# alv-around/mini-stark

Measured on AMD Instinct MI355X. Metric: stark_proofs_per_s, higher is better.
Workload: dtype u64; 1 GPU; Fibonacci AIR, Goldilocks, 2^20 trace rows, blowup 8, 20 security bits (w=3, c=6, rounds=23, ood_queries=1, fri_queries=2); a step = 8 independent proofs in flight per GPU

## Files before the change

mini-stark_amd/csrc/ctx.hpp:

```cpp
#pragma once
#include "../../include/ministark.h"

#include <cstdarg>
#include <cstdio>
#include <cstdlib>
#include <map>
#include <new>
#include <string>
#include <type_traits>
#include <vector>

#include "field.hpp"
#include "merkle.hpp"
#include "ntt.hpp"
#include "poly.hpp"

namespace msctx {

struct DevBuf {
  void* p = nullptr; size_t cap = 0;
  int ensure(size_t bytes) {
    if (bytes <= cap) return 0;
    if (p) msrt::free_dev(p);
    p = nullptr; cap = 0;
    size_t want = bytes + bytes / 8 + 256;
    if (msrt::malloc_dev(&p, want)) { p = nullptr; return 1; }
    cap = want;
    return 0;
  }
  void release() { if (p) msrt::free_dev(p); p = nullptr; cap = 0; }
// ... 112 lines not shown
  void drop_rccl();
  void unshard() { sh_on = false; sh_rank = 0; sh_world = 1; xs = xr = nullptr; xcap = 0; xfn = nullptr; xuser = nullptr; have_lde = false; nrounds_done = 0; blob_size = 0; }
  int set_shard_rccl(int rank, int world, const u8* unique_id, size_t cap) override;
  int rccl_selftest() override;
  int shard_proof_on_root(int on) override { proof_root_only = on ? 1 : 0; return MS_OK; }
  int shard_proof_is_elsewhere() const override { return (proof_root_only && sh_world > 1 && sh_rank != 0 && nrounds_done == fri_rounds && fri_rounds) ? 1 : 0; }
  int shard_round_is_distributed(int r) override { return (r >= 0 && (size_t)r < nrounds_done && rounds[r]->dist) ? 1 : 0; }
  int shard_stats(u64* out) override { if (!out) return fail(MS_ERR_ARG, "shard_stats"); memcpy(out, xstat, sizeof xstat); return MS_OK; }
  bool shardable(size_t leaf_groups) const { return sh_on && leaf_groups >= shard_min_leaves && leaf_groups >= (size_t)sh_world * (size_t)sh_world; }
  int set_shard(int rank, int world, void* d_send, void* d_recv, size_t cap, ms_exchange_fn fn, void* user) override;

  int fail_rt(int e, const char* what) { err = std::string("runtime error ") + std::to_string(e) + " in " + what + ": " + msrt::last_error_string(); return MS_ERR_HIP; }
  int fail(int code, const char* msg) { err = msg; return code; }

  enum { K_NTT_PASS, K_SCALE_POW, K_LEAF_HASH, K_INNER_HASH, K_TRANSPOSE, K_IO, K_LINCOMB, K_MIX, K_EVAL, K_EVAL_REDUCE, K_FOLD,
         K_SUFFIX_HORNER, K_DEGREE, K_FIND_FIRST, K_PATH, K_QUERY_POINTS, K_FRI_TAIL, K_COUNT };
  struct ProfRec { int kid, sub; msrt::Event* a; msrt::Event* b; double bytes; bool part; };
  int part_depth = 0;
  struct PartScope { Ctx* c; explicit PartScope(Ctx* c_) : c(c_) { c->part_depth++; } ~PartScope() { c->part_depth--; } };
  struct PartScopeIf { Ctx* c; bool on; PartScopeIf(Ctx* c_, bool on_) : c(c_), on(on_) { if (on) c->part_depth++; } ~PartScopeIf() { if (on) c->part_depth--; } };
  bool prof_on = false;
  std::vector<ProfRec> prof_recs;
  double next_bytes = 0;
  int next_sub = 0;
  std::vector<std::string> ntt_names{std::string("?")};
  void name_next(const char* fmt, ...) __attribute__((format(printf, 2, 3))) {
    if (!prof_on) return;
    char buf[200]; va_list ap; va_start(ap, fmt); vsnprintf(buf, sizeof buf, fmt, ap); va_end(ap);
    for (size_t i = 0; i < ntt_names.size(); i++) if (ntt_names[i] == buf) { next_sub = (int)i; return; }
    ntt_names.push_back(buf); next_sub = (int)ntt_names.size() - 1;
  }
// ... 23 lines not shown
    prof_recs.push_back(r);
    return e;
  }
  template <class K> int run(int kid, unsigned gx, unsigned gy, int threads, size_t lds, const typename K::Params& p) {
    launched();
    if (gx == 0 || gy == 0) return 0;
    if (!prof_on) return msrt::launch<K>(stream, gx, gy, threads, lds, p);
    ProfRec r; r.kid = kid; r.sub = next_sub; r.bytes = next_bytes; r.part = part_depth > 0; next_bytes = 0; next_sub = 0;
    if (msrt::event_create(&r.a) || msrt::event_create(&r.b)) return 1;
    msrt::event_record(r.a, stream);
    int e = msrt::launch<K>(stream, gx, gy, threads, lds, p);
    msrt::event_record(r.b, stream);
    prof_recs.push_back(r);
    return e;
  }
  int profile_begin() override { prof_on = true; return 0; }
  int profile_end(char* out, size_t cap) override;

  struct Plan {
    int log_n = 0, log_r0 = 0, log_rho = 0, npass = 0, K[4] = {0, 0, 0, 0}, lo_bits = 0;
    int LC[4] = {msntt::TILE_LOG_C, msntt::TILE_LOG_C, msntt::TILE_LOG_C, msntt::TILE_LOG_C};
    bool v2[4] = {false, false, false, false};
    bool regp[4] = {false, false, false, false};
    DevBuf tw_lo, tw_hi, w_r[4], vtw, w0;
    T n_inv = 0;
  };
  std::map<int, Plan*> plans;
  DevBuf ntt_scratch;
  int ntt_kmax = 9;
  int ntt_v2 = 1, ntt_v2_regpass = 1;
  int ntt_fast = 1;
// ... 182 lines not shown
  int sh_launch_inline(const SHJ& j, int final_mode);
  int sh_launch_table(const SHJ* d_jobs, size_t njobs, size_t maxnb, int final_mode);
  int shard_carry_table(const mspoly::CarryJob<F, E>* d_jobs, size_t njobs);
  int suffix_horner(const T* in, size_t in_limb_stride, size_t in_off, size_t in_stride, size_t m, const XE& z,
                    T* out, size_t out_limb_stride, size_t out_off, size_t out_stride, T* h0);

  int gather_poly(const T* local, size_t S, size_t count, T* dst, size_t dst_stride);
  int fold_dist(Round* pr, Round* nr, const XE& a, size_t* nq_coef_out);
  int fri_fold_commit(const u64* alpha, u8* root) override;
  size_t fri_tail_max = (size_t)1 << 15;
  int fri_overlap = 0;
  msrt::Stream* side_stream = nullptr; msrt::Event* ev_side = nullptr; bool side_pending = false;
  struct StreamScope { Ctx* c; msrt::Stream* keep; StreamScope(Ctx* c_, msrt::Stream* s) : c(c_), keep(c_->stream) { c->stream = s; } ~StreamScope() { c->stream = keep; } };
  int join_side() { if (side_pending) { side_pending = false; CK(msrt::stream_wait_event(stream, ev_side)); } return 0; }
  int fri_tail_round(Round* pr, Round* nr, const XE& a, bool* done);
  template <class DG> int fri_tail_round_t(Round* pr, Round* nr, const XE& a, bool* done);
  int fri_round_info(int r, u64* ncoef, u64* D) override;
  int fri_round_poly_read(int r, u64* out) override;
  int fri_round_codeword_read(int r, u64* out) override;

  bool blob_external = false;
  int fri_query(const u64* betas, int nq, u8* ext_out, size_t ext_cap, size_t* ext_len) override;
  struct QueryPlan {
    typedef mspoly::CarryJob<F, E> CJ; typedef mspoly::FindJob<F, E> FJ; typedef msmerkle::PathJob<F, E> PJ; typedef msmerkle::ShardPathJob<F, E> SPJ;
    size_t W = 0; int nq = 0; size_t pos = 0; u8* blob = nullptr;
    T* d_h0 = nullptr; T* d_tg = nullptr; unsigned long long* d_ix = nullptr;
    std::vector<size_t> rec_off, path_off; std::vector<u64> qlen; std::vector<T> x1h;
    std::vector<std::vector<SHJ>> tables; std::vector<int> table_mode, table_part; size_t n_agg_tables = 0;
    std::vector<CJ> carry_jobs; bool any_dist = false;
    std::vector<msmerkle::CopyJob> unp; std::vector<size_t> unp_first, unp_cnt, chunk_c0, chunk_len;
// ... 39 lines not shown
```

mini-stark_amd/csrc/fri_commit.cpp:

```cpp
#include "ctx.hpp"
#include "fri_tail.hpp"

namespace msctx {

template <class F>
int Ctx<F>::round_commit(Round* r, size_t ncoef_in, int nonzero_limbs, const Round* prev, const XE* alpha) {
  if (ctz64(r->D) > F::TWO_ADICITY) return fail(MS_ERR_SHAPE, "FRI domain larger than the field's two-adicity");
  RQ(tree_shape(r->D, 2, 2, &r->ts));
  r->m = 0;
  {
    const bool shard_next = shardable(r->D / 2);
    bool z_outside_base = false;
    for (int l = 1; l < E; l++) z_outside_base = z_outside_base || cur_z.c[l] != 0;
    if (prev && fri_pointwise && z_outside_base && prev->D == 2 * r->D && prev->ts.sharded == shard_next) {
      Plan* pl;
      RQ(get_plan(ctz64(prev->D), 0, false, &pl));
      const size_t W = (size_t)sh_world;
      const size_t m_out = shard_next ? r->D / (2 * W) : r->D;
      const size_t local = shard_next ? 2 * m_out : r->D;
      if (shard_next) r->m = m_out;
      if (r->cw.ensure(local * E * sizeof(T))) return fail(MS_ERR_NOMEM, "codeword");
      const size_t total = m_out * (shard_next ? 2 : 1);
      const XE c = e_add<F, E>(cur_B[0], e_mul<F>(cur_B[1], *alpha));
      auto fold_launch = [&](auto* kernel) {
        typedef typename std::remove_pointer<decltype(kernel)>::type FK;
        typename FK::Params fp;
        fp.src = prev->cw.template as<T>(); fp.src_limb_stride = shard_next ? 2 * prev->m : prev->D;
        fp.dst = r->cw.template as<T>(); fp.dst_limb_stride = local;
        fp.m_out = m_out; fp.log_m = (u32)ctz64(m_out); fp.groups = shard_next ? 2 : 1; fp.shard_W = shard_next ? (u32)W : 0; fp.shard_k = (u32)sh_rank;
        fp.tw_lo = pl->tw_lo.template as<T>(); fp.tw_hi = pl->tw_hi.template as<T>(); fp.lo_bits = (u32)pl->lo_bits; fp.log_D = (u32)ctz64(prev->D);
        fp.alpha = *alpha;
        fp.c2 = e_add<F, E>(c, c);
        fp.z = cur_z;
        fp.inv2 = f_inv<F>(F::from_u64(2));
        return run<FK>(K_FOLD, grid1(total, FK::THREADS * FK::ITEMS), 1, FK::THREADS, 0, fp);
      };
      next_bytes = (double)total * E * sizeof(T) * 3;
      { PartScopeIf part(this, shard_next); CK(total <= fold_small_max ? fold_launch((mspoly::FriFoldEvalKernel<F, E, 1>*)nullptr) : fold_launch((mspoly::FriFoldEvalKernel<F, E, 8>*)nullptr)); }
      if (shard_next) RQ((tree_build_sharded<E>(r->cw.template as<T>(), m_out, 1, 2 * m_out, 2, r->ts, r->nodes)));
      else RQ((tree_build<E>(r->cw.template as<T>(), 0, 1, r->D, 1, r->ts, r->nodes)));
      return 0;
    }
  }
  RQ(join_side());
  if (shardable(r->D / 2)) {
    const size_t m = r->D / (2 * (size_t)sh_world);
    r->m = m;
    if (r->cw.ensure(2 * m * E * sizeof(T))) return fail(MS_ERR_NOMEM, "codeword");
    const T* coef = r->poly.template as<T>(); size_t coef_stride = r->cap;
// ... 273 lines not shown
  u32 nl = 0; while (((size_t)1 << nl) < per) nl++;
  tp.sub.nodes = nr->nodes.template as<u32>(); tp.sub.child_off = 0; tp.sub.nchildren = M; tp.sub.ic = 2; tp.sub.nlevels = nl;
  u32 tl = 0; while (((size_t)1 << tl) < G) tl++;
  tp.top.nodes = nr->nodes.template as<u32>(); tp.top.child_off = 2 * M - 2 * G; tp.top.nchildren = G; tp.top.ic = 2; tp.top.nlevels = tl;
  tp.top.host_root = host_root(); tp.top.aux_src = dres; tp.top.aux_dst = reinterpret_cast<unsigned long long*>(pinned); tp.top.flag = arm_flag();
  tp.root_index = nr->ts.nodes - 1;
  tp.done = reinterpret_cast<u32*>(d_deg.as<u8>() + 128);
  next_bytes = (double)Dn * E * sizeof(T) * 3 + (double)M * 96;
  CK(run_coop<TK>(K_FRI_TAIL, (unsigned)(G + 1), TK::THREADS, TK::lds_bytes(), tp));
  root_on_host = true; aux_on_host = true;
  *done = true;
  return 0;
}

template <class F>
int Ctx<F>::fri_fold_commit(const u64* alpha, u8* root) {
  if (!have_deep) return fail(MS_ERR_STATE, "fri_fold_commit before fri_deep");
  XE a;
  if (!alpha || !root || !load_ext(alpha, &a)) return fail(MS_ERR_ARG, "alpha");
  Round* pr = rounds[nrounds_done - 1];
  if (pr->D < 4) return fail(MS_ERR_SHAPE, "FRI round domain too small to fold (merkle.rs:93-104 panics)");
  const size_t n = pr->ncoef, m = (n + 1) / 2;
  Round* nr = round_slot(nrounds_done);
  nr->cap = m ? m : 1;
  nr->D = pr->D / 2;
  nr->dist = false; nr->local_store = false; nr->S = 0;
  size_t nq_coef = 0;
  bool fused = false, side = false;
  RQ(fri_tail_round(pr, nr, a, &fused));
  if (fused) {
    CK(sync_results());
    nr->ncoef = (size_t)(*reinterpret_cast<unsigned long long*>(pinned));
    memcpy(root, reinterpret_cast<const u8*>(host_root()), 32);
    nrounds_done++; have_deep = false;
    return MS_OK;
  }
  if (pr->dist) RQ(fold_dist(pr, nr, a, &nq_coef));
  else {
  if (nr->poly.ensure(nr->cap * E * sizeof(T)) || d_folded.ensure((m + 1) * E * sizeof(T))) return fail(MS_ERR_NOMEM, "fold");
  if (m >= 2) {
    side = fri_overlap && !prof_on;
    if (side && !side_stream) { CK(msrt::stream_create(&side_stream)); CK(msrt::event_create(&ev_side)); }
    StreamScope on_side(this, side ? side_stream : stream);
    typename mspoly::FoldKernel<F, E>::Params fp{pr->poly.template as<T>(), pr->cap, n, d_folded.as<T>(), m, a, nullptr};
    CK(run<mspoly::FoldKernel<F, E>>(K_FOLD, grid1(m, mspoly::THREADS), 1, mspoly::THREADS, 0, fp));
    RQ(suffix_horner(d_folded.as<T>(), m, 0, 1, m, cur_z, nr->poly.template as<T>(), nr->cap, 0, 1, nullptr));
    nq_coef = m - 1;
  }
  }
  unsigned long long* dres = d_deg.as<unsigned long long>();
  if (nr->dist) {
    const size_t lc = lcount(nr, nq_coef);
    if (lc) {
      typename mspoly::DegreeKernel<F, E>::Params dp{lpoly(nr), lstride(nr), lc, dres, (size_t)sh_rank * nr->S};
      PartScope part(this);
      CK(run<mspoly::DegreeKernel<F, E>>(K_DEGREE, grid1(lc, mspoly::THREADS), 1, mspoly::THREADS, 0, dp));
    }
    shard_aux = dres;
  } else if (nq_coef) {
    StreamScope on_side(this, side ? side_stream : stream);
    typename mspoly::DegreeKernel<F, E>::Params dp{nr->poly.template as<T>(), nr->cap, nq_coef, dres, 0};
    CK(run<mspoly::DegreeKernel<F, E>>(K_DEGREE, grid1(nq_coef, mspoly::THREADS), 1, mspoly::THREADS, 0, dp));
  }
  if (side) { CK(msrt::event_record(ev_side, side_stream)); side_pending = true; }
  pending_aux = dres; aux_on_host = false;
  { auto clear = scope_exit([this] { pending_aux = nullptr; shard_aux = nullptr; });
    auto join = scope_exit([this] { if (side_pending) { side_pending = false; seq_armed = 0; msrt::stream_wait_event(stream, ev_side); } });
    RQ(round_commit(nr, nq_coef, E, pr, &a)); }
  if (!aux_on_host) { seq_armed = 0; CK(msrt::d2h(pinned, dres, 8, stream)); CK(msrt::memset_dev(dres, 0, 8, stream)); }
  if (!root_on_host) { seq_armed = 0; CK(msrt::d2h(reinterpret_cast<u8*>(pinned) + 64, nr->nodes.template as<u8>() + (nr->ts.local_nodes - 1) * 32, 32, stream)); }
  CK(sync_results());
  nr->ncoef = (size_t)(*reinterpret_cast<unsigned long long*>(pinned));
  memcpy(root, root_on_host ? reinterpret_cast<const u8*>(host_root()) : reinterpret_cast<const u8*>(pinned) + 64, 32);
  nrounds_done++; have_deep = false;
  return MS_OK;
}

template <class F>
int Ctx<F>::fri_round_info(int r, u64* ncoef, u64* D) {
  if (r < 0 || (size_t)r >= nrounds_done) return fail(MS_ERR_ARG, "round index");
  if (ncoef) *ncoef = rounds[r]->ncoef;
// ... 17 lines not shown

#define MS_INSTANTIATE(FF) \
  template int Ctx<FF>::round_commit(Ctx<FF>::Round* r, size_t ncoef_in, int nonzero_limbs, const Ctx<FF>::Round* prev, const Ctx<FF>::XE* alpha); \
  template int Ctx<FF>::degree_launch(const Ctx<FF>::T* poly, size_t limb_stride, size_t n, unsigned long long** dres_out); \
  template int Ctx<FF>::read_degree_and_root(const Ctx<FF>::T* poly, size_t limb_stride, size_t n, Ctx<FF>::Round* r, size_t* ncoef, u8* root); \
  template int Ctx<FF>::fri_begin(size_t blowup_, size_t nrounds, u8* root0); \
  template int Ctx<FF>::fri_deep(const u64* z, u64* B); \
  template Ctx<FF>::SHPlan Ctx<FF>::sh_plan(const Ctx<FF>::T* in, size_t in_limb_stride, size_t in_off, size_t in_stride, size_t m, const Ctx<FF>::XE& z, void* out, bool out_u64, size_t out_limb_stride, size_t out_off, size_t out_stride, Ctx<FF>::T* h0, Ctx<FF>::T* scratch, const Ctx<FF>::T* ext_carry, Ctx<FF>::T* top_agg, bool out_h0); \
  template int Ctx<FF>::sh_launch_inline(const Ctx<FF>::SHJ& j, int final_mode); \
  template int Ctx<FF>::sh_launch_table(const Ctx<FF>::SHJ* d_jobs, size_t njobs, size_t maxnb, int final_mode); \
  template int Ctx<FF>::shard_carry_table(const mspoly::CarryJob<FF, Ctx<FF>::E>* d_jobs, size_t njobs); \
  template int Ctx<FF>::suffix_horner(const Ctx<FF>::T* in, size_t in_limb_stride, size_t in_off, size_t in_stride, size_t m, const Ctx<FF>::XE& z, Ctx<FF>::T* out, size_t out_limb_stride, size_t out_off, size_t out_stride, Ctx<FF>::T* h0); \
  template int Ctx<FF>::gather_poly(const Ctx<FF>::T* local, size_t S, size_t count, Ctx<FF>::T* dst, size_t dst_stride); \
  template int Ctx<FF>::fold_dist(Ctx<FF>::Round* pr, Ctx<FF>::Round* nr, const Ctx<FF>::XE& a, size_t* nq_coef_out); \
  template int Ctx<FF>::fri_tail_round(Ctx<FF>::Round* pr, Ctx<FF>::Round* nr, const Ctx<FF>::XE& a, bool* done); \
  template int Ctx<FF>::fri_fold_commit(const u64* alpha, u8* root); \
  template int Ctx<FF>::fri_round_info(int r, u64* ncoef, u64* D); \
  template int Ctx<FF>::fri_round_poly_read(int r, u64* out); \
  template int Ctx<FF>::fri_round_codeword_read(int r, u64* out);
MS_INSTANTIATE(GL)
MS_INSTANTIATE(BB)
#undef MS_INSTANTIATE

}
```

mini-stark_amd/csrc/merkle_tree.cpp:

```cpp
#include "ctx.hpp"
#include "blake2s.hpp"

namespace msctx {

template <class F>
int Ctx<F>::tree_shape(size_t leaf_num, size_t lpn, size_t ic, TreeShape* ts) {
  if (lpn == 0 || ic < 2 || !is_pow2(ic)) return fail(MS_ERR_SHAPE, "merkle: bad leafs_per_node / inner_children");
  const size_t node_num = leaf_num / lpn;
  long lg = log_two_k(node_num, ic);
  if (lg < 0) return fail(MS_ERR_SHAPE, lg == -1 ? "number if not a power of 2" : "number if not a power of base");
  if (leaf_num % lpn != 0) return fail(MS_ERR_SHAPE, "merkle: leaf_num % leafs_per_node != 0");
  if (lg >= 64 || node_num == 0) return fail(MS_ERR_SHAPE, "Tree is not full!");
  ts->leaf_num = leaf_num; ts->lpn = lpn; ts->ic = ic; ts->levels = (size_t)lg + 1;
  size_t total = 0, m = node_num;
  for (;;) { total += m; if (m == 1) break; m /= ic; }
  ts->nodes = total; ts->local_nodes = total; ts->Mloc = 0; ts->sharded = false;
  return 0;
}

template <class F> template <int EL>
int Ctx<F>::leaf_hash(const T* base, size_t col_stride, size_t row_stride, size_t limb_stride, u32 width, size_t lpn, size_t ngroups, u32* out,
              size_t g_first, u32 run_len, u32 run_stride, const msmerkle::LinColSpec* lin, size_t out_g0) {
  if (ngroups >> 32) return fail(MS_ERR_SHAPE, "more than 2^32 leaf groups");
  if (digest == MS_DIGEST_BLAKE2S256) {
// ... 66 lines not shown
  auto to_rec = [&](msmerkle::InnerHashKernel::Params& ip) {
    ip.host_root = reinterpret_cast<u32*>(rec_out);
    if (shard_aux) { ip.aux_src = shard_aux; ip.aux_dst = reinterpret_cast<unsigned long long*>(rec_out + 32); }
    rec_done = true;
  };
  const bool b2 = digest == MS_DIGEST_BLAKE2S256;
  while (nchildren > 1) {
    msmerkle::InnerHashKernel::Params ip;
    ip.nodes = nodes; ip.child_off = child_off; ip.nchildren = nchildren; ip.ic = (u32)ic; ip.host_root = nullptr; ip.aux_src = nullptr; ip.aux_dst = nullptr; ip.flag = msrt::HostFlag{nullptr, 0};
    const size_t nparents = nchildren / ic;
    if (ic == 2 && nparents <= subtree_parents && (nchildren & (nchildren - 1)) == 0) {
      typedef msmerkle::InnerSubtreeKernel SK;
      u32 nl = 0; for (size_t m = nchildren; m > 1 && nl < (u32)SK::MAX_LEVELS; m >>= 1) nl++;
      const size_t left = nchildren >> nl;
      if (final_levels && left == 1) {
        RQ(join_side());
        ip.host_root = host_root(); root_on_host = true;
        if (pending_aux) { ip.aux_src = pending_aux; ip.aux_dst = reinterpret_cast<unsigned long long*>(pinned); pending_aux = nullptr; aux_on_host = true; }
        ip.flag = arm_flag();
      } else if (rec_out && left == 1) to_rec(ip);
      ip.nlevels = nl;
      next_bytes = (double)nchildren * 32 * 2;
      if (b2) CK(run_coop<msmerkle::B2InnerSubtreeKernel>(K_INNER_HASH, (unsigned)left, SK::THREADS, SK::lds_bytes(), ip));
      else CK(run_coop<SK>(K_INNER_HASH, (unsigned)left, SK::THREADS, SK::lds_bytes(), ip));
      for (u32 l = 0; l < nl; l++) { child_off += nchildren; nchildren >>= 1; }
      continue;
    }
    if (final_levels && (nparents == 1 || nparents <= (size_t)tree_top_parents)) {
      RQ(join_side());
      ip.host_root = host_root(); root_on_host = true;
      if (pending_aux) { ip.aux_src = pending_aux; ip.aux_dst = reinterpret_cast<unsigned long long*>(pinned); pending_aux = nullptr; aux_on_host = true; }
      ip.flag = arm_flag();
    } else if (rec_out && (nparents == 1 || nparents <= (size_t)tree_top_parents)) to_rec(ip);
    if (nparents <= (size_t)tree_top_parents) {
      u32 nl = 0; for (size_t m = nchildren; m > 1; m /= ic) nl++;
      ip.nlevels = nl;
      next_bytes = (double)nchildren * 32 * 2;
      RQ(inner_launch(1, ip));
      break;
    }
    ip.nlevels = 1;
    next_bytes = (double)nparents * (ic * 32 + 32);
    RQ(inner_launch((unsigned)((nparents + msmerkle::THREADS - 1) / msmerkle::THREADS), ip));
    child_off += nchildren; nchildren = nparents;
  }
  if (rec_out && !rec_done) {
    CK(msrt::d2d(rec_out, reinterpret_cast<u8*>(nodes) + (child_off + nchildren - 1) * 32, 32, stream));
    if (shard_aux) CK(msrt::d2d(rec_out + 32, shard_aux, 8, stream)); else CK(msrt::memset_dev(rec_out + 32, 0, 8, stream));
  }
  return 0;
}

template <class F> template <int EL>
int Ctx<F>::tree_build_sharded(const T* base, size_t col_stride, size_t row_stride, size_t limb_stride, u32 width, TreeShape& ts, DevBuf& nodes, const msmerkle::LinColSpec* lin) {
  const size_t W = (size_t)sh_world, M = ts.leaf_num / ts.lpn, Mloc = M / W, per = Mloc / W;
  if (ts.ic != 2 || per == 0) return fail(MS_ERR_STATE, "sharded tree needs a binary tree with at least world^2 leaf groups");
  if (Mloc * 32 > xcap) return fail(MS_ERR_NOMEM, "exchange buffers too small for the sharded commitment (need 32 * leaf groups / world bytes)");
  const size_t sub_nodes = 2 * Mloc - 1, top_nodes = 2 * W - 1;
// ... 110 lines not shown
```

mini-stark_amd/csrc/rt.hpp:

```cpp
#pragma once
#include <cstddef>
#include <cstdint>
#include <cstring>

#if defined(MS_HOST_ONLY)
#define MS_HD inline
#define MS_DEV inline
#define MS_RESTRICT
MS_HD uint64_t ms_mulhi64(uint64_t a, uint64_t b) { return (uint64_t)(((unsigned __int128)a * b) >> 64); }

#elif defined(MS_EMU)
#include <cstdlib>
#include <vector>
#define MS_HD inline
#define MS_DEV inline
#define MS_RESTRICT
namespace msrt {
struct Stream { int dummy; };
inline int malloc_dev(void** p, size_t n) { *p = std::malloc(n ? n : 1); return *p ? 0 : 1; }
inline int free_dev(void* p) { std::free(p); return 0; }
inline int malloc_host(void** p, size_t n) { *p = std::malloc(n ? n : 1); return *p ? 0 : 1; }
inline int malloc_host_coherent(void** p, size_t n) { return malloc_host(p, n); }
inline int free_host(void* p) { std::free(p); return 0; }
inline int h2d(void* d, const void* h, size_t n, Stream*) { std::memcpy(d, h, n); return 0; }
// ... 163 lines not shown
  return r;
}
template <class K> struct CoopArgs { const typename K::Params* p; int bx, by, nbx, threads; unsigned char* lds; };
template <class K> inline void coop_entry(void* a, int tid) { auto* c = (CoopArgs<K>*)a; K::run(*c->p, c->bx, c->by, c->nbx, tid, c->lds); }
template <class K>
inline int launch_coop(Stream*, unsigned gx, unsigned gy, int threads, size_t lds_bytes, const typename K::Params& p) {
  static thread_local FiberBlock fb;
  std::vector<unsigned char> lds(lds_bytes + 16);
  for (unsigned by = 0; by < gy; by++)
    for (unsigned bx = 0; bx < gx; bx++) {
      CoopArgs<K> a{&p, (int)bx, (int)by, (int)gx, threads, lds.data()};
      fb.run_block(threads, &coop_entry<K>, &a);
    }
  return 0;
}
MS_DEV void atomic_min_u64(unsigned long long* a, unsigned long long v) { if (v < *a) *a = v; }
MS_DEV void atomic_max_u64(unsigned long long* a, unsigned long long v) { if (v > *a) *a = v; }
MS_DEV unsigned atomic_add_u32(unsigned* a, unsigned v) { unsigned o = *a; *a = o + v; return o; }
MS_DEV unsigned wave_alloc_slot(unsigned* counter, bool want) { if (!want) return 0; unsigned o = *counter; *counter = o + 1; return o; }
MS_DEV bool wave_any(bool pred) { return pred; }
inline unsigned pair_swap(unsigned v) { return (unsigned)wave_shfl_xor(v, 7); }
inline unsigned pair_exchange_add(bool a_lane, unsigned v, unsigned t, unsigned s) {
  const unsigned long long r = wave_shfl_xor((unsigned long long)v | ((unsigned long long)t << 32), 7);
  return a_lane ? (unsigned)(r >> 32) + s : (unsigned)r + t;
}
inline unsigned rotr_var(unsigned x, unsigned r) { return (x >> r) | (x << ((32 - r) & 31)); }
struct HostFlag { unsigned long long* dst; unsigned long long val; };
MS_DEV void raise_host_flag(const HostFlag& f) { if (f.dst) *f.dst = f.val; }
inline void raise_host_flag_wg(const HostFlag& f, int tid) { if (f.dst && tid == 0) *f.dst = f.val; }
}
// ... 275 lines not shown
template <class K>
__global__ void __launch_bounds__(K::THREADS, MinWaves<K>::v) ms_kmain_coop(const typename K::Params p) {
  extern __shared__ __align__(16) unsigned char ms_lds[];
  K::run(p, (int)blockIdx.x, (int)blockIdx.y, (int)gridDim.x, (int)threadIdx.x, ms_lds);
}
template <class K>
inline int launch_coop(Stream* s, unsigned gx, unsigned gy, int threads, size_t lds_bytes, const typename K::Params& p) {
  if (threads != K::THREADS) return (int)hipErrorInvalidValue;
  if (lds_bytes > 65536) {
    hipError_t e = hipFuncSetAttribute(reinterpret_cast<const void*>(&ms_kmain_coop<K>), hipFuncAttributeMaxDynamicSharedMemorySize, (int)lds_bytes);
    if (e != hipSuccess) return (int)e;
  }
  hipLaunchKernelGGL(HIP_KERNEL_NAME(ms_kmain_coop<K>), dim3(gx, gy, 1), dim3(threads, 1, 1), lds_bytes, s, p);
  return (int)hipGetLastError();
}

MS_DEV void wg_barrier() { asm volatile("s_waitcnt lgkmcnt(0)\n\ts_barrier" ::: "memory"); }
MS_DEV void wg_barrier_global() { __syncthreads(); }
MS_DEV void fence_device() { __threadfence(); }
MS_DEV unsigned long long wave_shfl_xor(unsigned long long v, int mask) { return __shfl_xor(v, mask, 64); }
MS_DEV int wave_uniform(int v) { return __builtin_amdgcn_readfirstlane(v); }
MS_DEV void atomic_min_u64(unsigned long long* a, unsigned long long v) { atomicMin(a, v); }
MS_DEV void atomic_max_u64(unsigned long long* a, unsigned long long v) { atomicMax(a, v); }
MS_DEV unsigned atomic_add_u32(unsigned* a, unsigned v) { return atomicAdd(a, v); }
MS_DEV bool wave_any(bool pred) { return __any(pred) != 0; }
MS_DEV unsigned wave_alloc_slot(unsigned* counter, bool want) {
  const unsigned long long mask = __ballot(want);
  if (!want) return 0;
  const unsigned lane = __lane_id();
  const int leader = __ffsll((long long)mask) - 1;
// ... 51 lines not shown
```

mini-stark_amd/csrc/session.cpp:

```cpp
#include "ctx.hpp"

namespace msctx {

template <class F>
int Ctx<F>::profile_end(char* out, size_t cap) {
  static const char* names[K_COUNT] = {"ntt_pass", "scale_pow", "leaf_hash", "inner_hash", "transpose_in", "io_copy", "lincomb", "mix", "eval", "eval_reduce",
                                       "fold", "suffix_horner", "degree", "find_first", "merkle_path", "query_points", "fri_tail"};
  msrt::sync(stream);
  double ms[K_COUNT] = {0}, by[K_COUNT] = {0}, ms_part = 0, ms_repl = 0, repl_by[K_COUNT] = {0}; unsigned long long cnt[K_COUNT] = {0};
  std::map<int, double> sub_ms, sub_by; std::map<int, unsigned long long> sub_cnt;
  for (auto& r : prof_recs) {
    float t = 0.f; msrt::event_elapsed_ms(&t, r.a, r.b);
    ms[r.kid] += t; by[r.kid] += r.bytes; cnt[r.kid]++;
    if (r.part) ms_part += t; else { ms_repl += t; repl_by[r.kid] += t; }
    if (r.kid == K_NTT_PASS) { sub_ms[r.sub] += t; sub_by[r.sub] += r.bytes; sub_cnt[r.sub]++; }
    msrt::event_destroy(r.a); msrt::event_destroy(r.b);
  }
  prof_recs.clear(); prof_on = false;
  std::string j = "{";
  for (int k = 0; k < K_COUNT; k++) {
    char buf[256];
    snprintf(buf, sizeof buf, "%s\"%s\": {\"launches\": %llu, \"ms\": %.6f, \"alg_bytes\": %.0f}", k ? ", " : "", names[k], cnt[k], ms[k], by[k]);
    j += buf;
  }
  j += ", \"ntt_pass_variants\": {";
  bool first = true;
  for (auto& kv : sub_ms) {
    const int sub = kv.first; char buf[420];
    const char* name = ntt_names[(size_t)sub < ntt_names.size() ? sub : 0].c_str();
    snprintf(buf, sizeof buf, "%s\"%s\": {\"launches\": %llu, \"ms\": %.6f, \"alg_bytes\": %.0f}", first ? "" : ", ", name, sub_cnt[sub], kv.second, sub_by[sub]);
    j += buf; first = false;
  }
  j += "}";
// ... 58 lines not shown
  digest = (flags & MS_FLAG_DIGEST_BLAKE2S) ? MS_DIGEST_BLAKE2S256 : MS_DIGEST_SHA256;
  if (const char* e = getenv("MS_NTT_KMAX")) { int v = atoi(e); if (v >= 5 && v <= msntt::MAX_LOG_R) ntt_kmax = v; }
  if (const char* e = getenv("MS_NTT_FAST")) ntt_fast = atoi(e);
  if (const char* e = getenv("MS_NTT_V2")) ntt_v2 = atoi(e);
  if (const char* e = getenv("MS_NTT_V2_REGPASS")) ntt_v2_regpass = atoi(e);
  if (const char* e = getenv("MS_NTT_SHARE")) ntt_share = atoi(e);
  if (const char* e = getenv("MS_NTT_COOP_WGS")) { int v = atoi(e); if (v >= 8 && v <= 65536) ntt_coop_wgs = v & ~7; }
  if (const char* e = getenv("MS_LDE_LINEAR")) lde_linear = atoi(e);
  if (const char* e = getenv("MS_LAZY_LINCOMB")) lazy_lin = atoi(e);
  if (const char* e = getenv("MS_LDE_MULTI")) lde_multi = atoi(e);
  if (const char* e = getenv("MS_LDE_VIRTUAL")) lde_virtual = atoi(e);
  if (const char* e = getenv("MS_FRI_POINTWISE")) fri_pointwise = atoi(e);
  if (const char* e = getenv("MS_FOLD_SMALL_MAX")) fold_small_max = (size_t)atol(e);
  if (const char* e = getenv("MS_FRI_TAIL_MAX")) fri_tail_max = (size_t)atol(e);
  if (const char* e = getenv("MS_FRI_OVERLAP")) fri_overlap = atoi(e);
  if (const char* e = getenv("MS_SYNC_POLL")) poll_sync = atoi(e);
  if (const char* e = getenv("MS_EVAL_SMALL_MAX")) eval_small_max = (size_t)atol(e);
  if (const char* e = getenv("MS_TREE_SUBTREE_PARENTS")) subtree_parents = (size_t)atol(e);
  if (const char* e = getenv("MS_UPLOAD")) upload_sdma = !strcmp(e, "hip") ? 0 : 1;
  if (const char* e = getenv("MS_SDMA_TIMEOUT_S")) { const double v = atof(e); if (v > 0) sdma_timeout_s = v; }
  if (const char* e = getenv("MS_READBACK")) readback_sdma = !strcmp(e, "hip") ? 0 : (!strcmp(e, "sdma-async") ? 1 : 2);
  if (const char* e = getenv("MS_LEAF_LAZY_MIN")) leaf_lazy_min = atoi(e);
  if (const char* e = getenv("MS_TREE_TOP")) { int v = atoi(e); if (v >= 1 && v <= 65536) tree_top_parents = v; }
  if (const char* e = getenv("MS_SHARD_MIN_LEAVES")) { long v = atol(e); if (v >= 1) shard_min_leaves = (size_t)v; }
  if (const char* e = getenv("MS_SHARD_DIST")) shard_dist = atoi(e);
  if (const char* e = getenv("MS_SHARD_WORLD1")) allow_w1 = atoi(e);
  if (const char* e = getenv("MS_SHARD_STUB")) shard_stub = atoi(e);
  if (const char* e = getenv("MS_SHARD_GATHER_CHUNK")) { long v = atol(e); if (v >= 64) shard_gather_chunk = (size_t)v & ~(size_t)63; }
  if (const char* e = getenv("MS_SHARD_SLICES")) { int v = atoi(e); if (v >= 1 && v <= 64) { shard_slices = v; shard_slices_set = true; } }
  if (const char* e = getenv("MS_SHARD_SLICE_MIN")) { long v = atol(e); if (v >= 1) shard_slice_min = (size_t)v; }
// ... 162 lines not shown
```

Before: 275.2 proofs/s.

## Piggyback FRI fold, suffix-Horner scan and degree check onto Merkle hash launches

After: 277.8 proofs/s, median of 6. About the same (+0.9%).

```diff
diff --git a/mini-stark_amd/csrc/ctx.hpp b/mini-stark_amd/csrc/ctx.hpp
--- a/mini-stark_amd/csrc/ctx.hpp
+++ b/mini-stark_amd/csrc/ctx.hpp
@@ -14,6 +14,7 @@
 #include "merkle.hpp"
 #include "ntt.hpp"
 #include "poly.hpp"
+#include "fri_riders.hpp"
 
 namespace msctx {
 
@@ -156,7 +157,7 @@
   int fail(int code, const char* msg) { err = msg; return code; }
 
   enum { K_NTT_PASS, K_SCALE_POW, K_LEAF_HASH, K_INNER_HASH, K_TRANSPOSE, K_IO, K_LINCOMB, K_MIX, K_EVAL, K_EVAL_REDUCE, K_FOLD,
-         K_SUFFIX_HORNER, K_DEGREE, K_FIND_FIRST, K_PATH, K_QUERY_POINTS, K_FRI_TAIL, K_COUNT };
+         K_SUFFIX_HORNER, K_DEGREE, K_FIND_FIRST, K_PATH, K_QUERY_POINTS, K_FRI_TAIL, K_FRI_RIDER, K_COUNT };
   struct ProfRec { int kid, sub; msrt::Event* a; msrt::Event* b; double bytes; bool part; };
   int part_depth = 0;
   struct PartScope { Ctx* c; explicit PartScope(Ctx* c_) : c(c_) { c->part_depth++; } ~PartScope() { c->part_depth--; } };
@@ -210,7 +211,47 @@
     prof_recs.push_back(r);
     return e;
   }
-  int profile_begin() override { prof_on = true; return 0; }
+  typedef msfri::CoefRider<F, E> RiderK;
+  struct RiderSlot { bool on = false; unsigned nb = 0; typename RiderK::Params p; };
+  int fri_riders = 1;
+  RiderSlot ride_agg, ride_fin;
+  bool ride_agg_on_eval = false;
+  unsigned long long rider_phases = 0;
+  template <class H, bool HCOOP> int run_rider(int kid, RiderSlot& rs, unsigned gx, int threads, size_t lds, const typename H::Params& hp) {
+    rs.on = false;
+    if (gx == 0) { seq_armed = 0; seq_pending = 0; return fail(MS_ERR_STATE, "rider on an empty launch"); }
+    const size_t l2 = lds > RiderK::lds_bytes() ? lds : RiderK::lds_bytes();
+    ProfRec r; r.a = r.b = nullptr;
+    if (prof_on) {
+      r.kid = kid; r.sub = next_sub; r.bytes = next_bytes; r.part = part_depth > 0; next_bytes = 0; next_sub = 0;
+      if (msrt::event_create(&r.a) || msrt::event_create(&r.b)) { seq_armed = 0; seq_pending = 0; return 1; }
+      msrt::event_record(r.a, stream);
+    }
+    const int e = msrt::launch_rider<RiderK, H, HCOOP>(stream, rs.nb, rs.p, gx, threads, l2, hp);
+    if (e) { seq_armed = 0; seq_pending = 0; } else launched();
+    if (prof_on) { msrt::event_record(r.b, stream); prof_recs.push_back(r); if (!e) rider_phases++; }
+    return e;
+  }
+  int flush_riders() {
+    if (ride_agg.on) { ride_agg.on = false; CK(run_coop<RiderK>(K_SUFFIX_HORNER, ride_agg.nb, RiderK::THREADS, RiderK::lds_bytes(), ride_agg.p)); }
+    if (ride_fin.on) { ride_fin.on = false; CK(run_coop<RiderK>(K_SUFFIX_HORNER, ride_fin.nb, RiderK::THREADS, RiderK::lds_bytes(), ride_fin.p)); }
+    return 0;
+  }
+  bool tree_hosts_riders(size_t M, bool* level_before) const {
+    *level_before = false;
+    if (M < 2 || (M & (M - 1))) return false;
+    for (size_t nchildren = M; nchildren > 1; nchildren >>= 1) {
+      const size_t nparents = nchildren / 2;
+      if (nparents <= subtree_parents) {
+        u32 nl = 0; for (size_t m = nchildren; m > 1 && nl < (u32)msmerkle::InnerSubtreeKernel::MAX_LEVELS; m >>= 1) nl++;
+        return (nchildren >> nl) > 1;
+      }
+      if (nparents <= (size_t)tree_top_parents) return false;
+      *level_before = true;
+    }
+    return false;
+  }
+  int profile_begin() override { prof_on = true; rider_phases = 0; return 0; }
   int profile_end(char* out, size_t cap) override;
 
   struct Plan {
@@ -423,6 +464,7 @@
   struct StreamScope { Ctx* c; msrt::Stream* keep; StreamScope(Ctx* c_, msrt::Stream* s) : c(c_), keep(c_->stream) { c->stream = s; } ~StreamScope() { c->stream = keep; } };
   int join_side() { if (side_pending) { side_pending = false; CK(msrt::stream_wait_event(stream, ev_side)); } return 0; }
   int fri_tail_round(Round* pr, Round* nr, const XE& a, bool* done);
+  int plan_riders(Round* pr, Round* nr, const XE& a, bool* on);
   template <class DG> int fri_tail_round_t(Round* pr, Round* nr, const XE& a, bool* done);
   int fri_round_info(int r, u64* ncoef, u64* D) override;
   int fri_round_poly_read(int r, u64* out) override;
diff --git a/mini-stark_amd/csrc/fri_commit.cpp b/mini-stark_amd/csrc/fri_commit.cpp
--- a/mini-stark_amd/csrc/fri_commit.cpp
+++ b/mini-stark_amd/csrc/fri_commit.cpp
@@ -33,6 +33,9 @@
         fp.c2 = e_add<F, E>(c, c);
         fp.z = cur_z;
         fp.inv2 = f_inv<F>(F::from_u64(2));
+        if constexpr (FK::ITEMS == 1) {
+          if (ride_agg.on && ride_agg_on_eval) return run_rider<FK, false>(K_FOLD, ride_agg, grid1(total, FK::THREADS * FK::ITEMS), FK::THREADS, 0, fp);
+        }
         return run<FK>(K_FOLD, grid1(total, FK::THREADS * FK::ITEMS), 1, FK::THREADS, 0, fp);
       };
       next_bytes = (double)total * E * sizeof(T) * 3;
@@ -336,6 +339,42 @@
 }
 
 template <class F>
+int Ctx<F>::plan_riders(Round* pr, Round* nr, const XE& a, bool* on) {
+  *on = false;
+  ride_agg.on = false; ride_fin.on = false; ride_agg_on_eval = false;
+  const size_t n = pr->ncoef, m = (n + 1) / 2, M = nr->D / 2, BS = mspoly::SH_BS, nb = (m + BS - 1) / BS;
+  bool z_outside_base = false;
+  for (int l = 1; l < E; l++) z_outside_base = z_outside_base || cur_z.c[l] != 0;
+  if (!fri_riders || digest != MS_DIGEST_SHA256 || m < 2 || pr->dist || pr->ts.sharded || shardable(M) || !fri_pointwise || !z_outside_base || ctz64(nr->D) > F::TWO_ADICITY) return 0;
+  bool level_before = false;
+  if (!tree_hosts_riders(M, &level_before)) return 0;
+  if (nb > 512) return 0;
+  const bool two = nb > 1;
+  const size_t shared = sh_scratch_elems(m);
+  if (d_sh.ensure((shared + (two ? nb * nb * (size_t)E : 0)) * sizeof(T))) return fail(MS_ERR_NOMEM, "scan levels");
+  SHPlan sp = sh_plan(d_folded.as<T>(), m, 0, 1, m, cur_z, nr->poly.template as<T>(), false, nr->cap, 0, 1, nullptr, d_sh.as<T>());
+  if (sp.nl != (two ? 2 : 1)) return fail(MS_ERR_STATE, "rider scan plan");
+  typename RiderK::Params base;
+  memset(&base, 0, sizeof base);
+  base.fold = typename RiderK::FoldK::Params{pr->poly.template as<T>(), pr->cap, n, d_folded.as<T>(), m, a, nullptr};
+  base.deg = typename RiderK::DegK::Params{nr->poly.template as<T>(), nr->cap, m - 1, d_deg.as<unsigned long long>(), 0};
+  ride_fin.p = base; ride_fin.p.mode = RiderK::FINAL; ride_fin.nb = (unsigned)nb;
+  if (two) {
+    ride_agg.p = base; ride_agg.p.mode = RiderK::AGG; ride_agg.p.do_fold = 1; ride_agg.p.j1 = sp.agg[0]; ride_agg.nb = (unsigned)nb; ride_agg.on = true;
+    ride_agg_on_eval = !level_before;
+    T* priv = d_sh.as<T>() + shared;
+    ride_fin.p.do_top = 1; ride_fin.p.priv_stride = nb * (size_t)E;
+    ride_fin.p.j1 = sp.fin[1]; ride_fin.p.j1.out = priv;
+    ride_fin.p.j2 = sp.fin[0]; ride_fin.p.j2.carry = priv;
+  } else {
+    ride_fin.p.do_fold = 1; ride_fin.p.j2 = sp.fin[0];
+  }
+  ride_fin.on = true;
+  *on = true;
+  return 0;
+}
+
+template <class F>
 int Ctx<F>::fri_fold_commit(const u64* alpha, u8* root) {
   if (!have_deep) return fail(MS_ERR_STATE, "fri_fold_commit before fri_deep");
   XE a;
@@ -348,7 +387,9 @@
   nr->D = pr->D / 2;
   nr->dist = false; nr->local_store = false; nr->S = 0;
   size_t nq_coef = 0;
-  bool fused = false, side = false;
+  bool fused = false, side = false, riders = false;
+  bool side_open = false;
+  auto side_guard = scope_exit([&side_open, this] { if (side_open) { seq_armed = 0; if (!msrt::event_record(ev_side, side_stream)) msrt::stream_wait_event(stream, ev_side); } });
   RQ(fri_tail_round(pr, nr, a, &fused));
   if (fused) {
     CK(sync_results());
@@ -360,9 +401,12 @@
   if (pr->dist) RQ(fold_dist(pr, nr, a, &nq_coef));
   else {
   if (nr->poly.ensure(nr->cap * E * sizeof(T)) || d_folded.ensure((m + 1) * E * sizeof(T))) return fail(MS_ERR_NOMEM, "fold");
-  if (m >= 2) {
+  if (m >= 2) RQ(plan_riders(pr, nr, a, &riders));
+  if (m >= 2 && riders) nq_coef = m - 1;
+  else if (m >= 2) {
     side = fri_overlap && !prof_on;
     if (side && !side_stream) { CK(msrt::stream_create(&side_stream)); CK(msrt::event_create(&ev_side)); }
+    side_open = side;
     StreamScope on_side(this, side ? side_stream : stream);
     typename mspoly::FoldKernel<F, E>::Params fp{pr->poly.template as<T>(), pr->cap, n, d_folded.as<T>(), m, a, nullptr};
     CK(run<mspoly::FoldKernel<F, E>>(K_FOLD, grid1(m, mspoly::THREADS), 1, mspoly::THREADS, 0, fp));
@@ -379,14 +423,14 @@
       CK(run<mspoly::DegreeKernel<F, E>>(K_DEGREE, grid1(lc, mspoly::THREADS), 1, mspoly::THREADS, 0, dp));
     }
     shard_aux = dres;
-  } else if (nq_coef) {
+  } else if (nq_coef && !riders) {
     StreamScope on_side(this, side ? side_stream : stream);
     typename mspoly::DegreeKernel<F, E>::Params dp{nr->poly.template as<T>(), nr->cap, nq_coef, dres, 0};
     CK(run<mspoly::DegreeKernel<F, E>>(K_DEGREE, grid1(nq_coef, mspoly::THREADS), 1, mspoly::THREADS, 0, dp));
   }
-  if (side) { CK(msrt::event_record(ev_side, side_stream)); side_pending = true; }
+  if (side) { CK(msrt::event_record(ev_side, side_stream)); side_open = false; side_pending = true; }
   pending_aux = dres; aux_on_host = false;
-  { auto clear = scope_exit([this] { pending_aux = nullptr; shard_aux = nullptr; });
+  { auto clear = scope_exit([this] { pending_aux = nullptr; shard_aux = nullptr; ride_agg.on = false; ride_fin.on = false; });
     auto join = scope_exit([this] { if (side_pending) { side_pending = false; seq_armed = 0; msrt::stream_wait_event(stream, ev_side); } });
     RQ(round_commit(nr, nq_coef, E, pr, &a)); }
   if (!aux_on_host) { seq_armed = 0; CK(msrt::d2h(pinned, dres, 8, stream)); CK(msrt::memset_dev(dres, 0, 8, stream)); }
@@ -434,6 +478,7 @@
   template int Ctx<FF>::gather_poly(const Ctx<FF>::T* local, size_t S, size_t count, Ctx<FF>::T* dst, size_t dst_stride); \
   template int Ctx<FF>::fold_dist(Ctx<FF>::Round* pr, Ctx<FF>::Round* nr, const Ctx<FF>::XE& a, size_t* nq_coef_out); \
   template int Ctx<FF>::fri_tail_round(Ctx<FF>::Round* pr, Ctx<FF>::Round* nr, const Ctx<FF>::XE& a, bool* done); \
+  template int Ctx<FF>::plan_riders(Ctx<FF>::Round* pr, Ctx<FF>::Round* nr, const Ctx<FF>::XE& a, bool* on); \
   template int Ctx<FF>::fri_fold_commit(const u64* alpha, u8* root); \
   template int Ctx<FF>::fri_round_info(int r, u64* ncoef, u64* D); \
   template int Ctx<FF>::fri_round_poly_read(int r, u64* out); \
diff --git a/mini-stark_amd/csrc/fri_riders.hpp b/mini-stark_amd/csrc/fri_riders.hpp
--- /dev/null
+++ b/mini-stark_amd/csrc/fri_riders.hpp
@@ -0,0 +1,54 @@
+#pragma once
+#include "poly.hpp"
+
+namespace msfri {
+
+template <class F, int E> struct CoefRider {
+  typedef typename F::T T;
+  static constexpr int THREADS = mspoly::THREADS;
+  typedef mspoly::FoldKernel<F, E> FoldK;
+  typedef mspoly::SuffixHornerKernel<F, E> ScanK;
+  typedef mspoly::DegreeKernel<F, E> DegK;
+  static_assert(FoldK::THREADS == THREADS && ScanK::THREADS == THREADS && DegK::THREADS == THREADS, "one workgroup shape for every step");
+  enum { AGG = 0, FINAL = 1 };
+  struct Params {
+    u32 mode;
+    u32 do_fold, do_top;
+    typename FoldK::Params fold;
+    typename ScanK::Job j1;
+    typename ScanK::Job j2;
+    size_t priv_stride;
+    typename DegK::Params deg;
+  };
+  static MS_HD size_t lds_bytes() { return ScanK::lds_bytes(); }
+  static MS_DEV void run(const Params& p, int bx, int, int nbx, int tid, unsigned char* lds) {
+    if (p.do_fold) {
+      for (int k = 0; k < mspoly::SH_SEG; k++) FoldK::phase(0, p.fold, bx * mspoly::SH_SEG + k, 0, tid, THREADS, lds);
+      msrt::wg_barrier_global();
+    }
+    typename ScanK::Params sp;
+    sp.jobs = nullptr;
+    if (p.mode == AGG) { sp.inline_job = p.j1; sp.final_mode = 0; ScanK::run(sp, bx, 0, nbx, tid, lds); return; }
+    sp.final_mode = 1;
+    if (p.do_top) {
+      sp.inline_job = p.j1;
+      sp.inline_job.out = reinterpret_cast<T*>(p.j1.out) + (size_t)bx * p.priv_stride;
+      ScanK::run(sp, 0, 0, 1, tid, lds);
+      msrt::wg_barrier_global();
+    }
+    sp.inline_job = p.j2;
+    if (p.do_top) sp.inline_job.carry = p.j2.carry + (size_t)bx * p.priv_stride;
+    ScanK::run(sp, bx, 0, nbx, tid, lds);
+    msrt::wg_barrier_global();
+    const size_t BS = (size_t)mspoly::SH_BS;
+    const size_t lo = bx ? (size_t)bx * BS - 1 : 0;
+    size_t hi = ((size_t)bx + 1) * BS - 1;
+    if (hi > p.deg.n) hi = p.deg.n;
+    if (lo >= hi) return;
+    typename DegK::Params dp = p.deg;
+    dp.src = p.deg.src + lo; dp.n = hi - lo; dp.idx0 = p.deg.idx0 + lo;
+    for (int k = 0; (size_t)k * THREADS < dp.n; k++) DegK::phase(0, dp, k, 0, tid, THREADS, lds);
+  }
+};
+
+}
diff --git a/mini-stark_amd/csrc/merkle_tree.cpp b/mini-stark_amd/csrc/merkle_tree.cpp
--- a/mini-stark_amd/csrc/merkle_tree.cpp
+++ b/mini-stark_amd/csrc/merkle_tree.cpp
@@ -104,6 +104,7 @@
       u32 nl = 0; for (size_t m = nchildren; m > 1 && nl < (u32)SK::MAX_LEVELS; m >>= 1) nl++;
       const size_t left = nchildren >> nl;
       if (final_levels && left == 1) {
+        RQ(flush_riders());
         RQ(join_side());
         ip.host_root = host_root(); root_on_host = true;
         if (pending_aux) { ip.aux_src = pending_aux; ip.aux_dst = reinterpret_cast<unsigned long long*>(pinned); pending_aux = nullptr; aux_on_host = true; }
@@ -112,11 +113,16 @@
       ip.nlevels = nl;
       next_bytes = (double)nchildren * 32 * 2;
       if (b2) CK(run_coop<msmerkle::B2InnerSubtreeKernel>(K_INNER_HASH, (unsigned)left, SK::THREADS, SK::lds_bytes(), ip));
+      else if (ride_fin.on && left > 1) {
+        if (ride_agg.on) { ride_agg.on = false; CK(run_coop<RiderK>(K_SUFFIX_HORNER, ride_agg.nb, RiderK::THREADS, RiderK::lds_bytes(), ride_agg.p)); }
+        CK((run_rider<SK, true>(K_INNER_HASH, ride_fin, (unsigned)left, SK::THREADS, SK::lds_bytes(), ip)));
+      }
       else CK(run_coop<SK>(K_INNER_HASH, (unsigned)left, SK::THREADS, SK::lds_bytes(), ip));
       for (u32 l = 0; l < nl; l++) { child_off += nchildren; nchildren >>= 1; }
       continue;
     }
     if (final_levels && (nparents == 1 || nparents <= (size_t)tree_top_parents)) {
+      RQ(flush_riders());
       RQ(join_side());
       ip.host_root = host_root(); root_on_host = true;
       if (pending_aux) { ip.aux_src = pending_aux; ip.aux_dst = reinterpret_cast<unsigned long long*>(pinned); pending_aux = nullptr; aux_on_host = true; }
@@ -131,7 +137,9 @@
     }
     ip.nlevels = 1;
     next_bytes = (double)nparents * (ic * 32 + 32);
-    RQ(inner_launch((unsigned)((nparents + msmerkle::THREADS - 1) / msmerkle::THREADS), ip));
+    if (ride_agg.on && !ride_agg_on_eval && ic == 2 && !b2 && nparents / 2 <= subtree_parents)
+      CK((run_rider<msmerkle::InnerHashKernel2, false>(K_INNER_HASH, ride_agg, (unsigned)((nparents + msmerkle::THREADS - 1) / msmerkle::THREADS), msmerkle::THREADS, 0, ip)));
+    else RQ(inner_launch((unsigned)((nparents + msmerkle::THREADS - 1) / msmerkle::THREADS), ip));
     child_off += nchildren; nchildren = nparents;
   }
   if (rec_out && !rec_done) {
diff --git a/mini-stark_amd/csrc/rt.hpp b/mini-stark_amd/csrc/rt.hpp
--- a/mini-stark_amd/csrc/rt.hpp
+++ b/mini-stark_amd/csrc/rt.hpp
@@ -201,6 +201,13 @@
     }
   return 0;
 }
+template <class R, class H, bool HCOOP>
+inline int launch_rider(Stream* s, unsigned nr, const typename R::Params& rp, unsigned gx, int threads, size_t lds_bytes, const typename H::Params& hp) {
+  if (nr) { const int e = launch_coop<R>(s, nr, 1, threads, lds_bytes, rp); if (e) return e; }
+  if (!gx) return 0;
+  if constexpr (HCOOP) return launch_coop<H>(s, gx, 1, threads, lds_bytes, hp);
+  else return launch<H>(s, gx, 1, threads, lds_bytes, hp);
+}
 MS_DEV void atomic_min_u64(unsigned long long* a, unsigned long long v) { if (v < *a) *a = v; }
 MS_DEV void atomic_max_u64(unsigned long long* a, unsigned long long v) { if (v > *a) *a = v; }
 MS_DEV unsigned atomic_add_u32(unsigned* a, unsigned v) { unsigned o = *a; *a = o + v; return o; }
@@ -506,6 +513,29 @@
   hipLaunchKernelGGL(HIP_KERNEL_NAME(ms_kmain_coop<K>), dim3(gx, gy, 1), dim3(threads, 1, 1), lds_bytes, s, p);
   return (int)hipGetLastError();
 }
+template <class R, class H> struct RiderArgs { typename R::Params r; typename H::Params h; unsigned nr; };
+template <class R, class H, bool HCOOP>
+__global__ void __launch_bounds__(H::THREADS) ms_kmain_rider(const RiderArgs<R, H> a) {
+  static_assert(R::THREADS == H::THREADS, "rider and host share the workgroup shape");
+  extern __shared__ __align__(16) unsigned char ms_lds[];
+  const int nr = (int)a.nr, bx = (int)blockIdx.x;
+  if (bx < nr) { R::run(a.r, bx, 0, nr, (int)threadIdx.x, ms_lds); return; }
+  if constexpr (HCOOP) H::run(a.h, bx - nr, 0, (int)gridDim.x - nr, (int)threadIdx.x, ms_lds);
+  else {
+    const int nph = H::nphases(a.h);
+    for (int ph = 0; ph < nph; ph++) {
+      H::phase(ph, a.h, bx - nr, 0, (int)threadIdx.x, H::THREADS, ms_lds);
+      if (ph + 1 < nph) __syncthreads();
+    }
+  }
+}
+template <class R, class H, bool HCOOP>
+inline int launch_rider(Stream* s, unsigned nr, const typename R::Params& rp, unsigned gx, int threads, size_t lds_bytes, const typename H::Params& hp) {
+  if (threads != H::THREADS || lds_bytes > 65536) return (int)hipErrorInvalidValue;
+  RiderArgs<R, H> a; a.r = rp; a.h = hp; a.nr = nr;
+  hipLaunchKernelGGL(HIP_KERNEL_NAME(ms_kmain_rider<R, H, HCOOP>), dim3(nr + gx, 1, 1), dim3(threads, 1, 1), lds_bytes, s, a);
+  return (int)hipGetLastError();
+}
 
 MS_DEV void wg_barrier() { asm volatile("s_waitcnt lgkmcnt(0)\n\ts_barrier" ::: "memory"); }
 MS_DEV void wg_barrier_global() { __syncthreads(); }
diff --git a/mini-stark_amd/csrc/session.cpp b/mini-stark_amd/csrc/session.cpp
--- a/mini-stark_amd/csrc/session.cpp
+++ b/mini-stark_amd/csrc/session.cpp
@@ -5,7 +5,7 @@
 template <class F>
 int Ctx<F>::profile_end(char* out, size_t cap) {
   static const char* names[K_COUNT] = {"ntt_pass", "scale_pow", "leaf_hash", "inner_hash", "transpose_in", "io_copy", "lincomb", "mix", "eval", "eval_reduce",
-                                       "fold", "suffix_horner", "degree", "find_first", "merkle_path", "query_points", "fri_tail"};
+                                       "fold", "suffix_horner", "degree", "find_first", "merkle_path", "query_points", "fri_tail", "fri_rider"};
   msrt::sync(stream);
   double ms[K_COUNT] = {0}, by[K_COUNT] = {0}, ms_part = 0, ms_repl = 0, repl_by[K_COUNT] = {0}; unsigned long long cnt[K_COUNT] = {0};
   std::map<int, double> sub_ms, sub_by; std::map<int, unsigned long long> sub_cnt;
@@ -17,6 +17,7 @@
     msrt::event_destroy(r.a); msrt::event_destroy(r.b);
   }
   prof_recs.clear(); prof_on = false;
+  cnt[K_FRI_RIDER] = rider_phases; rider_phases = 0;
   std::string j = "{";
   for (int k = 0; k < K_COUNT; k++) {
     char buf[256];
@@ -105,6 +106,7 @@
   if (const char* e = getenv("MS_FOLD_SMALL_MAX")) fold_small_max = (size_t)atol(e);
   if (const char* e = getenv("MS_FRI_TAIL_MAX")) fri_tail_max = (size_t)atol(e);
   if (const char* e = getenv("MS_FRI_OVERLAP")) fri_overlap = atoi(e);
+  if (const char* e = getenv("MS_FRI_RIDERS")) fri_riders = atoi(e);
   if (const char* e = getenv("MS_SYNC_POLL")) poll_sync = atoi(e);
   if (const char* e = getenv("MS_EVAL_SMALL_MAX")) eval_small_max = (size_t)atol(e);
   if (const char* e = getenv("MS_TREE_SUBTREE_PARENTS")) subtree_parents = (size_t)atol(e);
```
